# facebookresearch/habitat-lab

Measured on AMD Instinct MI355X. Metric: env-steps/sec (SPS) PointNav RGB-D 256x256, 64 envs x 128 rollout, higher is better.
Workload: dtype f32; 1 GPU; PointNav SimpleCNN+GRU, 64 envs x 128 steps, 256x256 RGB-D synthetic; envs_per_gpu=64, rollout_steps=128, ppo_epoch=4, num_mini_batch=4, parallelism=dp1

## Files before the change

habitat-lab_amd/csrc/conv2_dgrad_strip.h:

```cpp
#pragma once
#include "igemm_bf3.h"
#include "ops.h"

namespace hab {

struct C2dArgs {
    const float* dy;
    const float* wd;
    const float* mask;
    float* dx;
    int B;
    int strips, items;
    int sign_schedule;
    int H, W, Ho, Wo;
};

template <int R2>
struct C2dCfg {
    static constexpr int H = 63, Ho = 30, Wo = 30, NT = 512, CELLS = 32;
    static constexpr int YRS = R2 + 1, YCOLS = 33, YPIX = YRS * YCOLS;
    static constexpr int YU = YRS * Wo * 16, YPT = (YU + NT - 1) / NT;
    static constexpr int Y_PLANE = YPIX * 64;
    static constexpr int RED_LD = 68;
    static constexpr size_t Y_BYTES = ((size_t)3 * Y_PLANE * 2 + 15) / 16 * 16, RED_BYTES = (size_t)8 * 32 * RED_LD * 4;
// ... 98 lines not shown
#pragma unroll
                for (int v = 0; v < 16; ++v) acc[pw][v] = 0.f;
#pragma unroll
            for (int j = 0; j < 4; ++j) {
                const unsigned short* src = ys + pixidx * 64 + (((2 * j + hi) ^ swz) << 3);
                bf16x8 yf[3];
#pragma unroll
                for (int pl = 0; pl < 3; ++pl) yf[pl] = *reinterpret_cast<const bf16x8*>(src + pl * Cfg::Y_PLANE);
                constexpr int PA[6] = {2, 0, 1, 1, 0, 0}, PB[6] = {0, 2, 1, 0, 1, 0};
#pragma unroll
                for (int q = 0; q < 6; ++q)
#pragma unroll
                    for (int pw = 0; pw < 2; ++pw)
                        acc[pw] = __builtin_amdgcn_mfma_f32_32x32x16_bf16(bw[j][pw][PB[q]], yf[PA[q]], acc[pw], 0, 0, 0);
            }
            if (tr > 0) __syncthreads();
            float* mine = red + (size_t)(wave * 32 + li) * Cfg::RED_LD;
#pragma unroll
            for (int pw = 0; pw < 2; ++pw)
#pragma unroll
                for (int g = 0; g < 4; ++g)
                    *reinterpret_cast<f32x4*>(mine + pw * 32 + 8 * g + 4 * hi) =
                        f32x4{acc[pw][4 * g], acc[pw][4 * g + 1], acc[pw][4 * g + 2], acc[pw][4 * g + 3]};
            __syncthreads();
            const int h2 = h20 + tr;
#pragma unroll
            for (int q = 0; q < 2; ++q) {
                const int idx = t + q * NT, rph = idx >> 9, cell = (idx >> 4) & 31, cq = idx & 15;
                f32x4 s = *reinterpret_cast<const f32x4*>(red + (size_t)(rph * 32 + cell) * Cfg::RED_LD + cq * 4);
#pragma unroll
                for (int t4 = 1; t4 < 4; ++t4)
                    s += *reinterpret_cast<const f32x4*>(red + (size_t)((2 * t4 + rph) * 32 + cell) * Cfg::RED_LD + cq * 4);
                if (flip) s = -s;
                const int h = 2 * h2 + rph, w = 2 * cell + (cq >> 3);
                if (h < H && w < W) {
                    const size_t off = (((size_t)img * H + h) * W + w) * 32 + (cq & 7) * 4;
                    if (a.mask) {
                        const f32x4 m = mk[q];
#pragma unroll
                        for (int e = 0; e < 4; ++e) s[e] = m[e] > 0.f ? s[e] : 0.f;
                    }
                    *reinterpret_cast<f32x4*>(a.dx + off) = s;
                }
            }
        }
        __syncthreads();
    }
}

inline bool conv2_dgrad_strip_covers(const ConvDesc& d) {
    return d.KH == 4 && d.KW == 4 && d.stride == 2 && d.pad == 0 && d.C == 32 && d.Cout == 64 && d.H >= 4 && d.W >= 4 && d.H <= 63 && d.W <= 63;
}

inline int conv2_dgrad_strip(const ConvDesc& d, const float* dy, const float* wd, const float* mask, const float* add, float* dx,
                             hipStream_t stream) {
    if (!conv2_dgrad_strip_covers(d)) return HAB_NOT_APPLICABLE;
    if (add || d.B < 16 || !dy || !wd || !dx) return HAB_NOT_APPLICABLE;
    if ((reinterpret_cast<uintptr_t>(dy) | reinterpret_cast<uintptr_t>(wd) | reinterpret_cast<uintptr_t>(dx) | reinterpret_cast<uintptr_t>(mask)) & 15) return HAB_NOT_APPLICABLE;
    constexpr int R2 = 2;
    using Cfg = C2dCfg<R2>;
    C2dArgs a;
    a.dy = dy; a.wd = wd; a.mask = mask; a.dx = dx; a.B = d.B;
    a.H = d.H; a.W = d.W; a.Ho = (d.H - 4) / 2 + 1; a.Wo = (d.W - 4) / 2 + 1;
    a.strips = ((d.H + 1) / 2 + R2 - 1) / R2;
    if ((long long)d.B * a.strips > 0x7fffffffLL) return HAB_NOT_APPLICABLE;
    a.items = d.B * a.strips;
    a.sign_schedule = bf3_sign_schedule();
    static const hipError_t attr_err = [] {
        const hipError_t e0 = hipFuncSetAttribute(reinterpret_cast<const void*>(conv2_dgrad_strip_kernel<R2, false>),
                                                  hipFuncAttributeMaxDynamicSharedMemorySize, (int)Cfg::LDS_BYTES);
        const hipError_t e1 = hipFuncSetAttribute(reinterpret_cast<const void*>(conv2_dgrad_strip_kernel<R2, true>),
                                                  hipFuncAttributeMaxDynamicSharedMemorySize, (int)Cfg::LDS_BYTES);
        return e0 != hipSuccess ? e0 : e1;
    }();
    if (attr_err != hipSuccess) return (int)attr_err;
    int grid = 256;
    while (grid > 8 && grid > a.items) grid -= 8;
    if (d.H == 63 && d.W == 63) conv2_dgrad_strip_kernel<R2, false><<<grid, Cfg::NT, Cfg::LDS_BYTES, stream>>>(a);
    else conv2_dgrad_strip_kernel<R2, true><<<grid, Cfg::NT, Cfg::LDS_BYTES, stream>>>(a);
    HAB_LAUNCH_CHECK();
    return HAB_OK;
}

}
```

habitat-lab_amd/csrc/gemm_ops.hip:

```cpp
#include "igemm.h"
#include "igemm_dma.h"
#include "igemm_dma_wgrad.h"
#include "igemm_bf3.h"
#include "igemm_bf3_ws.h"
#include "dense_bf3.h"
#include "obs_conv_bf3.h"
#include "obs_conv_bf3_ws.h"
#include "obs_conv_patch.h"
#include "wgrad3x3_bf3.h"
#include "conv2_fwd_strip.h"
#include "conv2_dgrad_strip.h"
#include "obs_wgrad_bf3.h"
#include "obs_wgrad_strip.h"
#include "conv_patch_bf3.h"
#include "wgrad3x3_patch.h"
#include "prob_build.h"
#include <stdlib.h>

#include <atomic>

#include "../../include/habitat_amd.h"

namespace hab {

static std::atomic<int> g_bf3_mode{-1};
int matrix_path_bits() {
    int m = g_bf3_mode.load(std::memory_order_relaxed);
    if (m < 0) {
        static const int from_env = hab_env_int("HAB_BF3", MP_DEFAULT);
        int expected = -1;
        g_bf3_mode.compare_exchange_strong(expected, from_env, std::memory_order_relaxed);
        m = g_bf3_mode.load(std::memory_order_relaxed);
    }
    return m;
}
extern "C" int hab_set_matrix_path(int mode) {
    const int prev = matrix_path_bits();
    if (mode >= 0) g_bf3_mode.store(mode, std::memory_order_relaxed);
    return prev;
}

template <int TM_, int TN_, int WM_, int WN_>
struct Tile {
    static constexpr int TM = TM_, TN = TN_, WM = WM_, WN = WN_;
};
using Tile128x128 = Tile<2, 2, 2, 2>;
static bool rows_fit(int M, int rows, int other) { return M % rows == 0 || cdiv(M, rows) * rows < cdiv(M, other) * other; }
template <bool WG, class F>
static int by_width(int M, int N, F launch) {
    if (N <= 32) {
        if constexpr (WG) {
            if (rows_fit(M, 96, 256)) return launch(Tile<1, 1, 3, 1>{});
        }
        return launch(Tile<2, 1, 4, 1>{});
    }
    if (N <= 64) {
        if constexpr (WG) {
            if (rows_fit(M, 96, 128)) return launch(Tile<1, 2, 3, 1>{});
        }
        return launch(Tile<1, 2, 4, 1>{});
    }
    return launch(Tile128x128{});
}

// ... 31 lines not shown
        if (p.dma_ok() && p.M > 64 && p.N <= 128) return dma_launch<true>(p, ws, ws_floats, target_blocks, stream);
    }
    if (p.M <= 64) {
        if (p.N <= 32) return igemm_launch<P, 1, 1, 2, 1>(p, ws, ws_floats, target_blocks, stream);
        if (p.N <= 64) return igemm_launch<P, 1, 1, 2, 2>(p, ws, ws_floats, target_blocks, stream);
        return igemm_launch<P, 1, 2, 2, 2>(p, ws, ws_floats, target_blocks, stream);
    }
    return by_width<WG>(p.M, p.N, [&](auto t) {
        using T = decltype(t);
        return igemm_launch<P, T::TM, T::TN, T::WM, T::WN>(p, ws, ws_floats, target_blocks, stream);
    });
}

static bool patch3x3_wanted(const ConvDesc& d, int M) { return matrix_path_on(MP_PATCH3X3) && d.stride == 1 && d.KH == 3 && d.KW == 3 && M > 64; }
static PatchGeom patch3x3_geom(const float* in, int Hi, int Wi, int Ci, int Ho, int Wo, int off, int flip) {
    PatchGeom gq{};
    gq.in = in; gq.Hi = Hi; gq.Wi = Wi; gq.Ci = Ci; gq.Ho = Ho; gq.Wo = Wo; gq.KH = 3; gq.KW = 3;
    gq.off_h = off; gq.off_w = off; gq.flip = flip;
    return gq;
}

int conv_fwd(const ConvDesc& d, const float* x, const float* wf, const float* bias, float* y, int relu, float* ws,
             size_t ws_floats, hipStream_t stream) {
    ConvFwdProb p;
    HAB_TRY(build(p, d, x, wf, bias, y, relu));
    if (matrix_path_on(MP_CONV2_FWD | MP_RC))
        HAB_TRY_FORM(conv2_fwd_strip(p, ws, ws_floats, stream));
    if (patch3x3_wanted(d, p.M))
        HAB_TRY_FORM(conv_patch_bf3_dispatch(p, patch3x3_geom(x, d.H, d.W, d.C, p.g.Ho, p.g.Wo, -d.pad, 0), ws, ws_floats, stream));
    return run_igemm(p, ws, ws_floats, stream);
}
int64_t obs_conv_weight_image_floats() { return ((int64_t)OCP_W_ELEMS + 1) / 2 + 4; }
int obs_conv_weight_image(const float* wf, int Cout, int KH, int KW, int C, void* img, hipStream_t stream) {
    return obs_conv_patch_weight_image(wf, Cout, KH, KW, C, reinterpret_cast<unsigned short*>(img), stream);
}
int obs_conv_fwd(const ConvDesc& d, const ObsView& obs, const float* wf, const float* bias, float* y, int relu, float* ws,
                 size_t ws_floats, hipStream_t stream, const void* wimg) {
    ObsConvFwdProb p;
    HAB_TRY(build(p, d, obs, wf, bias, y, relu));
    if (matrix_path_on(MP_OBS_PATCH | MP_OBS) && p.quad)
        HAB_TRY_FORM(obs_conv_patch_launch(p, ws, ws_floats, stream, reinterpret_cast<const unsigned short*>(wimg)));
    if (matrix_path_on(MP_WS | MP_OBS) && p.quad && p.M > 64)
        HAB_TRY_FORM(obs_conv_bf3_ws_launch(p, ws, ws_floats, stream));
    if (matrix_path_on(MP_OBS) && p.quad && p.M > 64)
        HAB_TRY_FORM(obs_conv_bf3_launch<2>(p, ws, ws_floats, stream));
    return run_igemm(p, ws, ws_floats, stream);
}
__global__ void dgrad_empty_class_kernel(ConvDgradProb p) {
    const long long total = (long long)p.g.B * p.Hc * p.Wc * p.N;
    for (long long e = (long long)blockIdx.x * blockDim.x + threadIdx.x; e < total; e += (long long)gridDim.x * blockDim.x)
        p.store((int)(e / p.N), (int)(e % p.N), 0.f);
}

int conv_dgrad(const ConvDesc& d, const float* dy, const float* wd, const float* mask, const float* add, float* dx,
               float* ws, size_t ws_floats, hipStream_t stream) {
    if (matrix_path_on(MP_CONV2_DGRAD | MP_RC))
        HAB_TRY_FORM(conv2_dgrad_strip(d, dy, wd, mask, add, dx, stream));
    if (d.stride > 1) {
        ConvDgradMergedProb q;
        HAB_TRY(check_conv(d));
        q.g = make_geom(d);
        if (ConvDgradMergedProb::applicable(q.g)) {
            q.dy = dy; q.w = wd; q.mask = mask; q.add = add; q.dx = dx;
            q.finish();
            if (matrix_path_on(MP_RC) && q.M > 64)
                return by_width<false>(q.M, q.N, [&](auto t) { return bf3_launch<ConvDgradMergedProb, decltype(t)>(q, ws, ws_floats, 256, stream); });
            if (q.dma_ok()) return dma_launch<false>(q, ws, ws_floats, 1024, stream);
        }
    }
    for (int ph = 0; ph < d.stride; ++ph)
        for (int pw = 0; pw < d.stride; ++pw) {
            ConvDgradProb p;
            HAB_TRY(build(p, d, dy, wd, mask, add, dx, ph, pw));
            if (p.Hc <= 0 || p.Wc <= 0) continue;
            if (patch3x3_wanted(d, p.M) && p.K > 0) {
                const int rc = conv_patch_bf3_dispatch(p, patch3x3_geom(dy, p.g.Ho, p.g.Wo, d.Cout, d.H, d.W, d.pad - 2, 1), ws, ws_floats, stream);
                if (rc == HAB_OK) continue;
                if (rc != HAB_NOT_APPLICABLE) return rc;
            }
            if (p.K <= 0) {
                p.M = d.B * p.Hc * p.Wc;
                dgrad_empty_class_kernel<<<1024, 256, 0, stream>>>(p);
                HAB_LAUNCH_CHECK();
                continue;
            }
            HAB_TRY(run_igemm(p, ws, ws_floats, stream));
        }
    return HAB_OK;
}
int conv_wgrad(const ConvDesc& d, const float* x, const float* dy, float* dw_oihw, float* dbias, float* ws, size_t ws_floats,
               hipStream_t stream) {
    ConvWgradProb p;
    HAB_TRY(build(p, d, x, dy, dw_oihw, dbias));
    if (ws && matrix_path_on(MP_WGRAD_STRIP | MP_IJ_WGRAD) && wgrad3x3_bf3_shape(p))
        HAB_TRY_FORM(wgrad3x3_bf3(p, ws, ws_floats, stream));
    if (ws && !matrix_path_on(MP_IJ_WGRAD)) {
        ConvWgradProb q = p;
        q.colsum = nullptr;
        auto bias_grad = [&] { return dbias ? colsum(dy, p.N, p.K, p.N, dbias, 0, ws, ws_floats, stream) : HAB_OK; };
        if (wgrad3x3_patch_ok(p)) {
            HAB_TRY(bias_grad());
            return wgrad3x3_patch(q, ws, ws_floats, stream);
        }
        if (d.pad == 0 && p.N <= 32 && wgrad_dma_ok(q)) {
            HAB_TRY(bias_grad());
            if (rows_fit(q.M, 288, 256)) return igemm_dma_wgrad_launch<3, 3, 1>(q, ws, ws_floats, 1024, stream);
            return igemm_dma_wgrad_launch<2, 4, 1>(q, ws, ws_floats, 1024, stream);
        }
    }
    return run_igemm(p, ws, ws_floats, stream);
// ... 194 lines not shown
        const int c = (int)(e % ld);
        const long long r = e / ld;
        wp[e] = c < C ? w[r * C + c] : 0.f;
    }
}
int pad_rows(const float* w, float* wp, int R, int C, int ld, hipStream_t stream) {
    if (!w || !wp || R <= 0 || C <= 0 || ld < C) return HAB_ERR_ARG;
    const long long total = (long long)R * ld;
    pad_rows_kernel<<<(int)fmin(2048.0, (double)cdivl(total, 256)), 256, 0, stream>>>(w, wp, R, C, ld);
    HAB_LAUNCH_CHECK();
    return HAB_OK;
}
int transpose2d(const float* w, float* wt, int R, int C, hipStream_t stream) {
    if (!w || !wt || R <= 0 || C <= 0) return HAB_ERR_ARG;
    transpose_kernel<<<dim3(cdiv(C, 32), cdiv(R, 32)), dim3(32, 8), 0, stream>>>(w, wt, R, C);
    HAB_LAUNCH_CHECK();
    return HAB_OK;
}

}

using namespace hab;

static ConvDesc mk(int B, int H, int W, int C, int Cout, int KH, int KW, int stride, int pad) {
    ConvDesc d;
    d.B = B; d.H = H; d.W = W; d.C = C; d.Cout = Cout; d.KH = KH; d.KW = KW; d.stride = stride; d.pad = pad;
    return d;
}
static ObsView mkobs(const uint8_t* rgb, const float* depth, const int* rows, int H, int W) {
    ObsView o;
    o.rgb = rgb; o.depth = depth; o.rows = rows; o.H = H; o.W = W; o.C = (rgb ? 3 : 0) + (depth ? 1 : 0);
    return o;
}

extern "C" int hab_conv2d_fwd(const float* x, const float* w_fwd, const float* bias, float* y, int B, int H, int W, int C,
                              int Cout, int KH, int KW, int stride, int pad, int relu, float* ws, size_t ws_floats,
                              hipStream_t stream) {
    if (!x || !w_fwd || !y) return HAB_ERR_ARG;
    return conv_fwd(mk(B, H, W, C, Cout, KH, KW, stride, pad), x, w_fwd, bias, y, relu, ws, ws_floats, stream);
}
extern "C" int hab_obs_conv2d_fwd(const uint8_t* rgb, const float* depth, const int* rows, const float* w_fwd,
                                  const float* bias, float* y, int B, int H, int W, int Cout, int KH, int KW, int stride,
                                  int pad, int relu, float* ws, size_t ws_floats, hipStream_t stream) {
    if ((!rgb && !depth) || !w_fwd || !y) return HAB_ERR_ARG;
    ObsView o = mkobs(rgb, depth, rows, H, W);
    return obs_conv_fwd(mk(B, H, W, o.C, Cout, KH, KW, stride, pad), o, w_fwd, bias, y, relu, ws, ws_floats, stream);
}
extern "C" int hab_conv2d_dgrad(const float* dy, const float* w_dgrad, const float* relu_mask, const float* add, float* dx,
                                int B, int H, int W, int C, int Cout, int KH, int KW, int stride, int pad, float* ws,
                                size_t ws_floats, hipStream_t stream) {
    if (!dy || !w_dgrad || !dx) return HAB_ERR_ARG;
    return conv_dgrad(mk(B, H, W, C, Cout, KH, KW, stride, pad), dy, w_dgrad, relu_mask, add, dx, ws, ws_floats, stream);
}
extern "C" int hab_conv2d_wgrad(const float* x, const float* dy, float* dw_oihw, float* dbias, int B, int H, int W, int C, int Cout,
                                int KH, int KW, int stride, int pad, float* ws, size_t ws_floats, hipStream_t stream) {
    if (!x || !dy || !dw_oihw) return HAB_ERR_ARG;
    return conv_wgrad(mk(B, H, W, C, Cout, KH, KW, stride, pad), x, dy, dw_oihw, dbias, ws, ws_floats, stream);
}
extern "C" int hab_obs_conv2d_wgrad(const uint8_t* rgb, const float* depth, const int* rows, const float* dy, float* dw_oihw,
                                    float* dbias, int B, int H, int W, int Cout, int KH, int KW, int stride, int pad, float* ws,
                                    size_t ws_floats, hipStream_t stream) {
    if ((!rgb && !depth) || !dy || !dw_oihw) return HAB_ERR_ARG;
    ObsView o = mkobs(rgb, depth, rows, H, W);
    return obs_conv_wgrad(mk(B, H, W, o.C, Cout, KH, KW, stride, pad), o, dy, dw_oihw, dbias, ws, ws_floats, stream);
}
extern "C" int hab_obs_conv2d_wgrad_form(const uint8_t* rgb, const float* depth, const int* rows, const float* dy, float* dw_oihw,
                                         float* dbias, int B, int H, int W, int Cout, int KH, int KW, int stride, int pad, const float* ws,
                                         size_t ws_floats) {
    if ((!rgb && !depth) || !dy || !dw_oihw) return HAB_ERR_ARG;
    ObsView o = mkobs(rgb, depth, rows, H, W);
    ObsConvWgradProb p;
    const int r = build(p, mk(B, H, W, o.C, Cout, KH, KW, stride, pad), o, dy, dw_oihw, dbias);
    if (r != HAB_OK) return r;
    return choose_obs_wgrad(p, ws, ws_floats);
}
extern "C" int hab_linear_fwd(const float* x, int ldx, const float* w, int ldw, const float* bias, float* y, int ldy, int M,
                              int N, int K, int relu, int accumulate, float* ws, size_t ws_floats, hipStream_t stream) {
    return linear_fwd(x, ldx, w, ldw, bias, y, ldy, M, N, K, relu, accumulate, ws, ws_floats, stream);
}
extern "C" int hab_linear_dgrad(const float* dy, int lddy, const float* w, int ldw, const float* relu_mask, int ldmask,
                                float* dx, int lddx, int M, int n_in, int n_out, int accumulate, float* ws, size_t ws_floats,
                                hipStream_t stream) {
    return linear_dgrad(dy, lddy, w, ldw, relu_mask, ldmask, n_in, dx, lddx, M, n_in, n_out, accumulate, ws, ws_floats, stream);
}
extern "C" int hab_linear_wgrad(const float* dy, int lddy, const float* x, int ldx, float* dw, int lddw, int M, int n_out,
                                int n_in, int perm_c, int perm_hw, int accumulate, float* ws, size_t ws_floats,
                                hipStream_t stream) {
    return linear_wgrad(dy, lddy, x, ldx, dw, lddw, M, n_out, n_in, perm_c, perm_hw, accumulate, ws, ws_floats, stream);
}
extern "C" int hab_debug_dense_trace(long long* out320) {
    return (int)hipMemcpyFromSymbol(out320, HIP_SYMBOL(hab::dn_trace), sizeof(long long) * 8 * 8 * 5);
}
extern "C" int hab_colsum(const float* a, int lda, int M, int N, float* out, int accumulate, float* ws, size_t ws_floats,
                          hipStream_t stream) {
    return colsum(a, lda, M, N, out, accumulate, ws, ws_floats, stream);
}
extern "C" int hab_repack_conv_weight(const float* w_oihw, float* w_fwd, float* w_dgrad, int Cout, int Cin, int KH, int KW,
                                      int cin_padded, hipStream_t stream) {
    return repack_conv(w_oihw, w_fwd, w_dgrad, Cout, Cin, KH, KW, cin_padded, stream);
}
extern "C" int hab_repack_flatten_weight(const float* w, float* w_packed, int N, int C, int HW, hipStream_t stream) {
    return repack_flatten(w, w_packed, N, C, HW, stream);
}
extern "C" int hab_transpose2d(const float* w, float* wt, int R, int C, hipStream_t stream) {
    return transpose2d(w, wt, R, C, stream);
}
// ... 1 lines not shown
```

habitat-lab_amd/habitat_amd/_lib.py:

```python
from __future__ import annotations

import ctypes as C
import os
from ctypes import POINTER, c_char_p, c_double, c_float, c_int, c_int32, c_int64, c_size_t, c_uint8, c_uint32, c_void_p

_HERE = os.path.dirname(os.path.abspath(__file__))
LIB_PATH = os.path.join(_HERE, "libhabitat_amd.so")

vp = c_void_p
ALLREDUCE_FN = C.CFUNCTYPE(None, c_void_p, c_int, c_float, c_void_p)
GRAD_READY_FN = C.CFUNCTYPE(None, c_int64, c_int64, c_void_p)


class HabError(RuntimeError):
    pass


class PolicyDesc(C.Structure):
    _fields_ = [(n, c_int32) for n in (
        "arch", "backbone", "baseplanes", "normalize_visual_inputs", "rnn_type", "rnn_layers", "hidden", "num_actions",
        "H", "W", "has_rgb", "has_depth", "goal_dim", "max_frames", "max_envs", "visual_order", "has_semantic",
        "num_object_categories", "has_compass", "has_gps", "action_dist", "gauss_flags")] + [("gauss_min_std", c_float),
                                                                                                ("gauss_max_std", c_float),
                                                                                                ("pointgoal_dim", c_int32),
# ... 18 lines not shown
                ("gps", vp), ("visual_features", vp), ("pointgoal", vp), ("proximity", vp), ("visual", vp * 4), ("fused", vp * 8)]


class EmbedSlot(C.Structure):
    _fields_ = [("kind", c_int32), ("input", vp), ("weight", vp), ("bias", vp), ("d_weight", vp), ("d_bias", vp), ("num_tokens", c_int32)]


class PackInfo(C.Structure):
    _fields_ = [("select_inds", vp), ("frag_env", vp), ("frag_start", vp), ("step_offsets_host", vp),
                ("num_seqs_at_step_host", vp), ("P", c_int32), ("F", c_int32), ("max_len", c_int32), ("env_first_frame", vp)]


SIGNATURES = {
    "hab_abi_version": (c_int, []),
    "hab_error_string": (c_char_p, [c_int]),
    "hab_synth_step": (c_int, [vp, vp, vp, vp, vp, vp, vp, c_uint32, c_uint32, c_int, c_int, c_int, c_int, vp]),
    "hab_synth_objectnav_sensors": (c_int, [vp, vp, vp, vp, vp, c_uint32, c_uint32, c_int, c_int, c_int, vp]),
    "hab_nav2d_state_bytes": (c_int, []),
    "hab_nav2d_step": (c_int, [vp] * 13 + [c_uint32, c_uint32] + [c_int] * 7 + [vp]),
    "hab_nav2d_vel_step": (c_int, [vp] * 13 + [c_uint32, c_uint32] + [c_int] * 8 + [c_float, c_int, c_int, vp]),
    "hab_nav2d_geo_bytes": (c_int, []),
    "hab_nav2d_geo_build": (c_int, [vp, c_size_t, vp, vp, c_int, c_int, c_int, vp]),
    "hab_nav2d_step_geo": (c_int, [vp] * 14 + [c_uint32, c_uint32] + [c_int] * 7 + [vp]),
    "hab_nav2d_vel_step_geo": (c_int, [vp] * 14 + [c_uint32, c_uint32] + [c_int] * 8 + [c_float, c_int, c_int, vp]),
    "hab_nav2d_obj_state_bytes": (c_int, []),
    "hab_nav2d_obj_step": (c_int, [vp] * 17 + [c_uint32, c_uint32] + [c_int] * 10 + [vp]),
    "hab_nav2d_obj_geo_bytes": (c_int, []),
    "hab_nav2d_obj_geo_build": (c_int, [vp, c_size_t, vp, vp, c_int, c_int, c_int, c_int, vp]),
    "hab_nav2d_obj_step_geo": (c_int, [vp] * 18 + [c_uint32, c_uint32] + [c_int] * 10 + [vp]),
    "hab_nav2d_rearr_state_bytes": (c_int, []),
    "hab_nav2d_rearr_step": (c_int, [vp] * 15 + [c_uint32, c_uint32] + [c_int] * 8 + [vp]),
    "hab_obs_resize_crop": (c_int, [vp, vp, c_int, c_int, c_int, c_int, c_int, c_int, c_int, c_int, c_int, c_int, c_int, c_int, vp]),
    "hab_obs_resize_crop_form": (c_int, [vp, c_int, c_int, c_int, c_int, c_int, c_int, c_int, c_int]),
    "hab_obs_project": (c_int, [vp, c_int, vp, c_int, c_int, c_int, c_int, c_int, vp, vp, c_int, c_int, vp]),
    "hab_rollout_step_stats": (c_int, [vp, vp, vp, vp, vp, vp, vp, c_int, c_int, vp]),
    "hab_compute_returns": (c_int, [vp, vp, vp, vp, vp, c_int, c_int, c_float, c_float, c_int, c_int, vp]),
    "hab_advantages": (c_int, [vp, vp, vp, c_int, c_int, vp, vp, vp]),
    "hab_ppo_loss": (c_int, [vp, vp, vp, vp, vp, vp, vp, vp, c_int, c_float, c_float, c_float, c_int, vp, vp, vp, vp, vp]),
    "hab_ppo_loss_ver": (c_int, [vp, vp, vp, vp, vp, vp, vp, vp, c_int, c_float, c_float, c_float, c_int, vp, vp, vp, c_int64, vp, c_float,
                                 vp, vp, vp, vp, vp]),
    "hab_lagrange_adam_step": (c_int, [vp, vp, vp, vp, c_float, c_float, c_float, c_float, c_float, c_int, c_float, c_float, vp, vp]),
    "hab_ver_compute_returns": (c_int, [vp, vp, vp, vp, vp, vp, vp, vp, c_int, c_double, c_double, vp]),
    "hab_ver_is_coeffs": (c_int, [vp, c_int, c_int, c_int, vp, vp, vp]),
    "hab_clip_adam_step": (c_int, [vp, vp, vp, vp, c_size_t, vp, c_int, c_float, c_float, c_float, c_float, c_float,
                                   c_float, c_int, vp, vp]),
    "hab_sample_actions": (c_int, [vp, vp, vp, c_int, c_int, c_int, vp]),
    "hab_set_matrix_path": (c_int, [c_int]),
    "hab_conv2d_fwd": (c_int, [vp, vp, vp, vp] + [c_int] * 10 + [vp, c_size_t, vp]),
    "hab_obs_conv2d_fwd": (c_int, [vp, vp, vp, vp, vp, vp] + [c_int] * 9 + [vp, c_size_t, vp]),
    "hab_conv2d_dgrad": (c_int, [vp, vp, vp, vp, vp] + [c_int] * 9 + [vp, c_size_t, vp]),
    "hab_conv2d_wgrad": (c_int, [vp, vp, vp, vp] + [c_int] * 9 + [vp, c_size_t, vp]),
    "hab_obs_conv2d_wgrad": (c_int, [vp, vp, vp, vp, vp, vp] + [c_int] * 8 + [vp, c_size_t, vp]),
    "hab_obs_conv2d_wgrad_form": (c_int, [vp, vp, vp, vp, vp, vp] + [c_int] * 8 + [vp, c_size_t]),
    "hab_linear_fwd": (c_int, [vp, c_int, vp, c_int, vp, vp, c_int, c_int, c_int, c_int, c_int, c_int, vp, c_size_t, vp]),
    "hab_linear_dgrad": (c_int, [vp, c_int, vp, c_int, vp, c_int, vp, c_int, c_int, c_int, c_int, c_int, vp, c_size_t, vp]),
    "hab_linear_wgrad": (c_int, [vp, c_int, vp, c_int, vp, c_int, c_int, c_int, c_int, c_int, c_int, c_int, vp, c_size_t, vp]),
    "hab_colsum": (c_int, [vp, c_int, c_int, c_int, vp, c_int, vp, c_size_t, vp]),
    "hab_repack_conv_weight": (c_int, [vp, vp, vp, c_int, c_int, c_int, c_int, c_int, vp]),
    "hab_repack_flatten_weight": (c_int, [vp, vp, c_int, c_int, c_int, vp]),
    "hab_transpose2d": (c_int, [vp, vp, c_int, c_int, vp]),
    "hab_obs_ingest_pool": (c_int, [vp, vp, vp, vp, vp, c_int, c_int, c_int, c_int, c_int, c_int, c_int, vp]),
    "hab_obs_ingest_pool_sensors": (c_int, [vp, vp, vp, vp, c_int, vp, vp, c_int, c_int, c_int, c_int, vp, vp, vp, vp, vp, vp]),
    "hab_fused_gather": (c_int, [vp, vp, c_int, vp, vp, c_int, c_int, c_int, c_int, c_int, vp]),
    "hab_channel_moments": (c_int, [vp, c_int64, c_int, c_int, vp, vp, vp, c_int, vp]),
    "hab_running_mean_var_update": (c_int, [vp, vp, vp, vp, vp, c_float, c_int, vp]),
    "hab_running_mean_var_normalize": (c_int, [vp, c_int64, c_int, c_int, vp, vp, vp]),
    "hab_groupnorm_fwd": (c_int, [vp, vp, vp, vp, vp, vp, vp, c_int, c_int, c_int, c_int, c_int, c_float, vp, c_int64, vp]),
    "hab_groupnorm_bwd": (c_int, [vp, vp, vp, vp, vp, vp, vp, vp, vp, c_int, c_int, c_int, c_int, vp, c_int64, vp]),
    "hab_split_weight_planes": (c_int, [vp, c_int, c_int, vp, vp]),
    "hab_stem_split_weights": (c_int, [vp, vp, vp]),
    "hab_stem_conv_wgrad": (c_int, [vp, vp, vp, c_int, c_int, c_int, c_int, vp, c_size_t, vp, vp]),
    "hab_stem_conv_fwd": (c_int, [vp, vp, vp, c_int, c_int, c_int, vp, vp, c_int, vp]),
    "hab_conv_gn_fwd": (c_int, [vp] * 9 + [c_int] * 11 + [c_float, vp]),
    "hab_maxpool3x3s2_fwd": (c_int, [vp, vp, vp, c_int, c_int, c_int, c_int, vp]),
    "hab_maxpool3x3s2_bwd": (c_int, [vp, vp, vp, c_int, c_int, c_int, c_int, vp]),
    "hab_nav_embed_fwd": (c_int, [POINTER(EmbedSlot), c_int, vp, vp, vp, c_int, c_int, c_int, vp, vp]),
    "hab_nav_embed_bwd": (c_int, [POINTER(EmbedSlot), c_int, vp, vp, c_int, c_int, c_int, vp, c_size_t, vp]),
    "hab_build_pack_info": (c_int, [vp, c_int, c_int] + [vp] * 12),
    "hab_build_pack_info_from_ids": (c_int, [vp, vp, vp, c_int] + [vp] * 11),
    "hab_policy_create": (c_int, [POINTER(PolicyDesc), POINTER(vp)]),
    "hab_policy_destroy": (None, [vp]),
    "hab_policy_num_params": (c_int, [vp]),
    "hab_policy_param_info": (c_int, [vp, c_int, c_char_p, c_int, POINTER(c_int64), POINTER(c_int), POINTER(c_int64)]),
    "hab_policy_param_is_buffer": (c_int, [vp, c_int]),
    "hab_policy_set_training": (c_int, [vp, c_int]),
    "hab_comm_available": (c_int, []),
    "hab_comm_unique_id": (c_int, [vp]),
    "hab_comm_create": (c_int, [vp, c_int, c_int, vp]),
    "hab_comm_destroy": (None, [vp]),
    "hab_comm_world_size": (c_int, [vp]),
    "hab_comm_allreduce_sum": (c_int, [vp, vp, c_int64, vp]),
    "hab_policy_set_comm": (c_int, [vp, vp]),
    "hab_policy_grad_sync": (c_int, [vp, vp]),
    "hab_policy_set_grad_ready": (c_int, [vp, GRAD_READY_FN, vp]),
    "hab_policy_set_allreduce": (c_int, [vp, ALLREDUCE_FN, vp, c_int]),
    "hab_policy_param_floats": (c_int64, [vp]),
    "hab_policy_packed_floats": (c_int64, [vp]),
    "hab_policy_work_floats": (c_int64, [vp]),
    "hab_policy_bind": (c_int, [vp, vp, vp, vp, vp, c_int64]),
    "hab_policy_repack": (c_int, [vp, vp]),
    "hab_policy_encode": (c_int, [vp, POINTER(Obs), c_int, vp, vp]),
    "hab_policy_visual_feature_shape": (c_int, [vp, POINTER(c_int), POINTER(c_int), POINTER(c_int)]),
    "hab_policy_act": (c_int, [vp, POINTER(Obs), vp, vp, vp, c_int, c_int, vp, vp, vp, vp, vp, vp]),
    "hab_policy_evaluate": (c_int, [vp, POINTER(Obs), vp, vp, c_int, vp, vp, POINTER(PackInfo), c_int, c_int, vp, vp, vp, vp]),
    "hab_policy_final_hidden": (c_int, [vp, vp, vp]),
    "hab_policy_set_extra_grads": (c_int, [vp, vp, vp]),
# ... 46 lines not shown
```

include/habitat_amd.h:

```cpp
#ifndef HABITAT_AMD_H
#define HABITAT_AMD_H

#include <stddef.h>
#include <stdint.h>

#ifdef __cplusplus
extern "C" {
#endif

#ifndef __HIP_PLATFORM_AMD__
typedef struct ihipStream_t* hipStream_t;
#endif

#define HAB_ABI_VERSION 1
int hab_abi_version(void);
const char* hab_error_string(int code);

int hab_synth_step(uint8_t* rgb , float* depth , float* goal , float* reward ,
                   uint8_t* not_done , int64_t* env_t , int64_t* since_reset , uint32_t seed,
                   uint32_t env_offset, int N, int H, int W, int advance, hipStream_t stream);
int hab_synth_objectnav_sensors(int32_t* semantic, int64_t* objectgoal, float* compass, float* gps, const int64_t* env_t,
                                uint32_t seed, uint32_t env_offset, int N, int H, int W, hipStream_t stream);

#define HAB_NAV2D_STATE_BYTES 224
// ... 124 lines not shown
#define HAB_ADV_EXT_NORMALIZE 3
#define HAB_ADV_STATS_VAR 4
int hab_advantages(const float* returns, const float* value_preds, float* adv, int count, int mode,
                   const float* ext_stats, float* stats_out, hipStream_t stream);

int hab_ppo_loss(const float* values, const float* logp, const float* entropy, const float* old_logp,
                 const float* adv, const float* old_values, const float* returns, const int* rows, int B,
                 float clip_param, float value_loss_coef, float entropy_coef, int use_clipped_value_loss,
                 float* d_value, float* d_logp, float* d_entropy, float* out12, hipStream_t stream);

int hab_ppo_loss_ver(const float* values, const float* logp, const float* entropy, const float* old_logp, const float* adv,
                     const float* old_values, const float* returns, const int* rows, int B, float clip_param, float value_loss_coef,
                     float entropy_coef, int use_clipped_value_loss, const float* is_coeffs, const uint8_t* is_stale,
                     const int64_t* policy_version, int64_t current_policy_version, const float* log_alpha, float entropy_threshold,
                     float* d_value, float* d_logp, float* d_entropy, float* out20, hipStream_t stream);
int hab_lagrange_adam_step(float* log_alpha, float* exp_avg, float* exp_avg_sq, const float* grad, float grad_scale, float lr, float beta1,
                           float beta2, float eps, int step, float log_alpha_min, float log_alpha_max,
                           float* alpha_out , hipStream_t stream);

int hab_ver_compute_returns(const float* rewards, const float* value_preds, const uint8_t* is_stale, float* returns,
                            const int32_t* select_inds, const int32_t* step_offsets, const int32_t* sequence_lengths,
                            const uint8_t* last_sequence_in_batch_mask, int F, double gamma, double tau, hipStream_t stream);
int hab_ver_is_coeffs(const int64_t* environment_ids, int n, int num_envs, int num_steps, int32_t* counts_scratch, float* is_coeffs,
                      hipStream_t stream);

int hab_clip_adam_step(float* params, const float* grads, float* exp_avg, float* exp_avg_sq, size_t n,
                       double* scratch_partials, int scratch_len, float grad_scale, float max_grad_norm, float lr,
                       float beta1, float beta2, float eps, int step, float* grad_norm_out, hipStream_t stream);

int hab_sample_actions(const float* probs, const float* exp_noise, int64_t* actions, int n, int A, int deterministic,
                       hipStream_t stream);

int hab_set_matrix_path(int mode);

int hab_conv2d_fwd(const float* x, const float* w_fwd, const float* bias, float* y, int B, int H, int W, int C, int Cout,
                   int KH, int KW, int stride, int pad, int relu, float* ws, size_t ws_floats, hipStream_t stream);
int hab_obs_conv2d_fwd(const uint8_t* rgb, const float* depth, const int* rows, const float* w_fwd, const float* bias,
                       float* y, int B, int H, int W, int Cout, int KH, int KW, int stride, int pad, int relu, float* ws,
                       size_t ws_floats, hipStream_t stream);
int hab_conv2d_dgrad(const float* dy, const float* w_dgrad, const float* relu_mask, const float* add, float* dx, int B,
                     int H, int W, int C, int Cout, int KH, int KW, int stride, int pad, float* ws, size_t ws_floats,
                     hipStream_t stream);
int hab_conv2d_wgrad(const float* x, const float* dy, float* dw_oihw, float* dbias, int B, int H, int W, int C, int Cout,
                     int KH, int KW, int stride, int pad, float* ws, size_t ws_floats, hipStream_t stream);
int hab_obs_conv2d_wgrad(const uint8_t* rgb, const float* depth, const int* rows, const float* dy, float* dw_oihw,
                         float* dbias, int B, int H, int W, int Cout, int KH, int KW, int stride, int pad, float* ws,
                         size_t ws_floats, hipStream_t stream);
#define HAB_OBS_WGRAD_FORM_IGEMM 0
#define HAB_OBS_WGRAD_FORM_IM2COL 1
#define HAB_OBS_WGRAD_FORM_STRIP 2
int hab_obs_conv2d_wgrad_form(const uint8_t* rgb, const float* depth, const int* rows, const float* dy, float* dw_oihw,
                              float* dbias, int B, int H, int W, int Cout, int KH, int KW, int stride, int pad, const float* ws,
                              size_t ws_floats);
int hab_linear_fwd(const float* x, int ldx, const float* w, int ldw, const float* bias, float* y, int ldy, int M, int N,
                   int K, int relu, int accumulate, float* ws, size_t ws_floats, hipStream_t stream);
int hab_linear_dgrad(const float* dy, int lddy, const float* w, int ldw, const float* relu_mask, int ldmask, float* dx,
                     int lddx, int M, int n_in, int n_out, int accumulate, float* ws, size_t ws_floats,
                     hipStream_t stream);
int hab_linear_wgrad(const float* dy, int lddy, const float* x, int ldx, float* dw, int lddw, int M, int n_out, int n_in,
                     int perm_c, int perm_hw, int accumulate, float* ws, size_t ws_floats, hipStream_t stream);
int hab_colsum(const float* a, int lda, int M, int N, float* out, int accumulate, float* ws, size_t ws_floats,
               hipStream_t stream);
int hab_repack_conv_weight(const float* w_oihw, float* w_fwd, float* w_dgrad, int Cout, int Cin, int KH, int KW,
                           int cin_padded, hipStream_t stream);
int hab_repack_flatten_weight(const float* w, float* w_packed, int N, int C, int HW, hipStream_t stream);
int hab_transpose2d(const float* w, float* wt, int R, int C, hipStream_t stream);

int hab_obs_ingest_pool(const uint8_t* rgb, const float* depth, const int32_t* semantic, const int* rows, float* y, int B, int H, int W,
                        int cpad, int c_rgb, int c_depth, int c_sem ,
                        hipStream_t stream);
int hab_obs_ingest_pool_sensors(const void* const* sensors, const int32_t* dtypes, const int32_t* channels, const float* scales, int n,
                                const int* rows, float* y, int B, int H, int W, int cpad, const float* norm_mean, const float* norm_var,
                                const float* pivot, double* mom_partial, int* mom_blocks, hipStream_t stream);
int hab_fused_gather(const float* const* sensors, const int32_t* widths, int n, const int* rows, float* dst, int ld, int col0, int pad0,
                     int npad, int B, hipStream_t stream);
int hab_channel_moments(const float* x, int64_t npix, int cpad, int mode, const float* mean, float* out, double* scratch,
                        int scratch_len, hipStream_t stream);
int hab_running_mean_var_update(float* r_mean, float* r_var, float* r_count, const float* b_mean, const float* b_var, float n, int C,
                                hipStream_t stream);
int hab_running_mean_var_normalize(float* x, int64_t npix, int cpad, int C, const float* mean, const float* var, hipStream_t stream);
int hab_groupnorm_fwd(const float* x, float* y, const float* gamma, const float* beta, const float* residual, float* mean,
                      float* rstd, int B, int HW, int C, int groups, int relu, float eps, float* ws, int64_t ws_floats,
                      hipStream_t stream);
int hab_groupnorm_bwd(const float* x, const float* dy, const float* relu_out, float* dx, float* dy_masked, const float* gamma,
                      const float* mean, const float* rstd, float* chan_sums, int B, int HW, int C, int groups, float* ws,
                      int64_t ws_floats, hipStream_t stream);
int hab_split_weight_planes(const float* w_fwd, int Cout, int K, uint16_t* planes, hipStream_t stream);
int hab_stem_split_weights(const float* w_fwd, uint16_t* planes, hipStream_t stream);
int hab_stem_conv_fwd(const float* x, const uint16_t* w_planes, float* y, int B, int H, int W, const float* norm, float* gn_part, int gn_groups,
                      hipStream_t stream);
int hab_stem_conv_wgrad(const float* x, const float* dy, float* dw_oihw, int B, int H, int W, int creal, float* ws, size_t ws_floats,
                        const float* norm, hipStream_t stream);
int hab_conv_gn_fwd(const float* x, const uint16_t* w_planes, const float* gamma, const float* beta, const float* residual, float* y,
                    float* raw, float* mean, float* rstd, int B, int H, int W, int C, int Cout, int KH, int KW, int stride, int pad,
                    int groups, int relu, float eps, hipStream_t stream);
int hab_maxpool3x3s2_fwd(const float* x, float* y, uint8_t* idx, int B, int H, int W, int C, hipStream_t stream);
int hab_maxpool3x3s2_bwd(const float* dy, const uint8_t* idx, float* dx, int B, int H, int W, int C, hipStream_t stream);
#define HAB_EMB_POLAR 0
#define HAB_EMB_TOKEN 1
#define HAB_EMB_COSSIN 2
#define HAB_EMB_LIN2 3
#define HAB_EMB_PREV 4
#define HAB_EMB_PREVLIN 5
#define HAB_EMB_LINN 6
typedef struct hab_embed_slot {
    int32_t kind;
// ... 182 lines not shown
```

Before: 63940 env-steps/s.

## Add strip-tiled MFMA dgrad kernel for the 3x3 stride-1 conv3 layer

Adds a dedicated dgrad kernel for the 3x3/stride-1, 64-to-32-channel conv layer. It stages dy row strips in LDS as three-way bf16-split planes, plus a sign-flipped copy for the sign schedule, and accumulates the nine taps with 32x32x16 bf16 MFMA across two wave groups that hand off partial sums through LDS. Work is distributed through per-XCD atomic draw counters taken from a device-side slot pool, replacing the generic implicit-GEMM dgrad path for this layer. It also factors out the applicability checks and exposes a form query, at the cost of extra code complexity and device-counter reset logic.

```diff
diff --git a/habitat-lab_amd/csrc/conv2_dgrad_strip.h b/habitat-lab_amd/csrc/conv2_dgrad_strip.h
--- a/habitat-lab_amd/csrc/conv2_dgrad_strip.h
+++ b/habitat-lab_amd/csrc/conv2_dgrad_strip.h
@@ -174,18 +174,23 @@
     return d.KH == 4 && d.KW == 4 && d.stride == 2 && d.pad == 0 && d.C == 32 && d.Cout == 64 && d.H >= 4 && d.W >= 4 && d.H <= 63 && d.W <= 63;
 }
 
+constexpr int C2D_CELL_ROWS = 2;
+inline bool conv2_dgrad_strip_serves(const ConvDesc& d, const float* dy, const float* wd, const float* mask, const float* add, const float* dx) {
+    if (!conv2_dgrad_strip_covers(d)) return false;
+    if (add || d.B < 16 || !dy || !wd || !dx) return false;
+    if ((reinterpret_cast<uintptr_t>(dy) | reinterpret_cast<uintptr_t>(wd) | reinterpret_cast<uintptr_t>(dx) | reinterpret_cast<uintptr_t>(mask)) & 15) return false;
+    return (long long)d.B * cdiv((d.H + 1) / 2, C2D_CELL_ROWS) <= 0x7fffffffLL;
+}
+
 inline int conv2_dgrad_strip(const ConvDesc& d, const float* dy, const float* wd, const float* mask, const float* add, float* dx,
                              hipStream_t stream) {
-    if (!conv2_dgrad_strip_covers(d)) return HAB_NOT_APPLICABLE;
-    if (add || d.B < 16 || !dy || !wd || !dx) return HAB_NOT_APPLICABLE;
-    if ((reinterpret_cast<uintptr_t>(dy) | reinterpret_cast<uintptr_t>(wd) | reinterpret_cast<uintptr_t>(dx) | reinterpret_cast<uintptr_t>(mask)) & 15) return HAB_NOT_APPLICABLE;
-    constexpr int R2 = 2;
+    if (!conv2_dgrad_strip_serves(d, dy, wd, mask, add, dx)) return HAB_NOT_APPLICABLE;
+    constexpr int R2 = C2D_CELL_ROWS;
     using Cfg = C2dCfg<R2>;
     C2dArgs a;
     a.dy = dy; a.wd = wd; a.mask = mask; a.dx = dx; a.B = d.B;
     a.H = d.H; a.W = d.W; a.Ho = (d.H - 4) / 2 + 1; a.Wo = (d.W - 4) / 2 + 1;
-    a.strips = ((d.H + 1) / 2 + R2 - 1) / R2;
-    if ((long long)d.B * a.strips > 0x7fffffffLL) return HAB_NOT_APPLICABLE;
+    a.strips = cdiv((d.H + 1) / 2, R2);
     a.items = d.B * a.strips;
     a.sign_schedule = bf3_sign_schedule();
     static const hipError_t attr_err = [] {
diff --git a/habitat-lab_amd/csrc/conv3_dgrad_strip.h b/habitat-lab_amd/csrc/conv3_dgrad_strip.h
--- /dev/null
+++ b/habitat-lab_amd/csrc/conv3_dgrad_strip.h
@@ -0,0 +1,241 @@
+#pragma once
+#include "igemm_bf3.h"
+#include "ops.h"
+
+#include <atomic>
+
+namespace hab {
+
+struct C3dArgs {
+    const float* dy;
+    const float* wd;
+    const float* mask;
+    float* dx;
+    int B;
+    int strips, items;
+    int sign_schedule;
+    int H, W, Ho, Wo;
+    unsigned* ctr;
+};
+
+constexpr int C3D_DRAW_SLOTS = 64;
+__device__ unsigned c3d_draw_pool[C3D_DRAW_SLOTS * 16];
+
+template <int R>
+struct C3dCfg {
+    static constexpr int H = 30, Ho = 28, Wo = 28, NT = 512, MAXWO = 30;
+    static constexpr int YRS = R + 2, YCOLS = 34, YPIX = YRS * YCOLS;
+    static constexpr int YU = YRS * Wo * 8, YPT = (YRS * MAXWO * 8 + NT - 1) / NT;
+    static constexpr int Y_PLANE = YPIX * 32;
+    static constexpr int Y_COPY = 3 * Y_PLANE;
+    static constexpr size_t Y_BYTES = (size_t)2 * Y_COPY * 2, PASS_BYTES = (size_t)2 * 4 * 16 * 64 * 4;
+    static constexpr size_t LDS_BYTES = Y_BYTES + PASS_BYTES;
+    static_assert(R % 2 == 0, "the waves take the rows of a strip in pairs");
+    static_assert((Y_COPY * 2) % 256 == 0, "both copies on the same banks");
+};
+
+template <int R, bool RT>
+__global__ void __launch_bounds__(512) conv3_dgrad_strip_kernel(const C3dArgs a) {
+    using Cfg = C3dCfg<R>;
+    constexpr int NT = Cfg::NT;
+    const int H = RT ? a.H : Cfg::H, W = RT ? a.W : Cfg::H, Ho = RT ? a.Ho : Cfg::Ho, Wo = RT ? a.Wo : Cfg::Wo;
+    const int YU = Cfg::YRS * Wo * 8;
+    extern __shared__ __attribute__((aligned(16))) unsigned short smem16[];
+    unsigned short* ys = smem16;
+    f32x4* pass = reinterpret_cast<f32x4*>(reinterpret_cast<char*>(smem16) + Cfg::Y_BYTES);
+    const int t = threadIdx.x, lane = t & 63;
+    const int wave = __builtin_amdgcn_readfirstlane(t >> 6);
+    const int rsel = wave & 1, chalf = (wave >> 1) & 1, z = wave >> 2;
+    const int li = lane & 31, hi = lane >> 5;
+
+    __shared__ int s_draw[2];
+    const int xcd = blockIdx.x & 7;
+    const int per_xcd = (a.items + 7) >> 3, run0 = xcd * per_xcd, run_len = max(0, min(a.items, run0 + per_xcd) - run0);
+    if (t == 0) { s_draw[0] = (int)atomicAdd(a.ctr + xcd, 1u); s_draw[1] = (int)atomicAdd(a.ctr + xcd, 1u); }
+
+    for (int i = t; i < (int)(Cfg::Y_BYTES / 16); i += NT) reinterpret_cast<u32x4*>(smem16)[i] = u32x4{0u, 0u, 0u, 0u};
+
+    bf16x8 bw[9][3];
+    int tapoff[9];
+#pragma unroll
+    for (int j = 0; j < 9; ++j) {
+        const int s = 9 * z + j, tap = s >> 1, coh = s & 1, kh = tap / 3, kw = tap - 3 * kh;
+        tapoff[j] = (2 - kh) * Cfg::YCOLS + 2 - kw;
+        const float* src = a.wd + ((size_t)(chalf * 32 + li) * 9 + tap) * 32 + coh * 16 + hi * 8;
+        const f32x4 v0 = *reinterpret_cast<const f32x4*>(src), v1 = *reinterpret_cast<const f32x4*>(src + 4);
+        unsigned p[3][4];
+        bf3_split2(v0[0], v0[1], p[0][0], p[1][0], p[2][0]);
+        bf3_split2(v0[2], v0[3], p[0][1], p[1][1], p[2][1]);
+        bf3_split2(v1[0], v1[1], p[0][2], p[1][2], p[2][2]);
+        bf3_split2(v1[2], v1[3], p[0][3], p[1][3], p[2][3]);
+#pragma unroll
+        for (int pl = 0; pl < 3; ++pl) bw[j][pl] = __builtin_bit_cast(bf16x8, u32x4{p[pl][0], p[pl][1], p[pl][2], p[pl][3]});
+    }
+
+    f32x4 yr[Cfg::YPT];
+    int pf_h0 = 0;
+    auto fetch = [&](int item) {
+        const int img = item / a.strips, h0 = (item - img * a.strips) * R;
+        pf_h0 = h0;
+#pragma unroll
+        for (int j = 0; j < Cfg::YPT; ++j) {
+            const int u = t + j * NT;
+            const int r = u / (Wo * 8), row = h0 - 2 + r;
+            const bool ok = u < YU && (unsigned)row < (unsigned)Ho;
+            const size_t off = ok ? ((size_t)img * Ho + row) * (size_t)(Wo * 32) + (size_t)(u - r * (Wo * 8)) * 4 : 0;
+            yr[j] = *reinterpret_cast<const f32x4*>(a.dy + off);
+        }
+    };
+    auto stage = [&]() {
+#pragma unroll
+        for (int j = 0; j < Cfg::YPT; ++j) {
+            const int u = t + j * NT;
+            if (u >= YU) continue;
+            const int r = u / (Wo * 8), rem = u - r * (Wo * 8), w = rem >> 3, c4 = rem & 7;
+            const int pixidx = r * Cfg::YCOLS + w + 2;
+            unsigned short* dst = ys + pixidx * 32 + (((c4 >> 1) ^ ((pixidx >> 2) & 3)) << 3) + (c4 & 1) * 4;
+            const bool in_image = (unsigned)(pf_h0 - 2 + r) < (unsigned)Ho;
+            const f32x4 v = in_image ? yr[j] : f32x4{0.f, 0.f, 0.f, 0.f};
+            unsigned w0[3], w1[3];
+            bf3_split2(v[0], v[1], w0[0], w0[1], w0[2]);
+            bf3_split2(v[2], v[3], w1[0], w1[1], w1[2]);
+#pragma unroll
+            for (int pl = 0; pl < 3; ++pl) {
+                *reinterpret_cast<u32x2*>(dst + pl * Cfg::Y_PLANE) = u32x2{w0[pl], w1[pl]};
+                *reinterpret_cast<u32x2*>(dst + Cfg::Y_COPY + pl * Cfg::Y_PLANE) = u32x2{w0[pl] ^ 0x80008000u, w1[pl] ^ 0x80008000u};
+            }
+        }
+    };
+
+    __syncthreads();
+    int cur = s_draw[0], nxt = s_draw[1];
+    if (cur < run_len) fetch(run0 + cur);
+    for (int it = 0; cur < run_len; ++it) {
+        const int item = run0 + cur;
+        stage();
+        __syncthreads();
+        const bool more = nxt < run_len;
+        if (more) fetch(run0 + nxt);
+        if (more && t == 0) s_draw[it & 1] = (int)atomicAdd(a.ctr + xcd, 1u);
+        const int img = item / a.strips, h0 = (item - img * a.strips) * R;
+#pragma unroll 1
+        for (int ph = 0; ph <= R / 2; ++ph) {
+            const int rp = ph - z;
+            if (rp >= 0 && rp < R / 2) {
+                const int tr = 2 * rp + rsel, h = h0 + tr;
+                const bool live = h < H && li < W;
+                const size_t out = (((size_t)img * H + h) * W + li) * 64 + chalf * 32 + 4 * hi;
+                const bool flip = a.sign_schedule && ((((img * H + h) * W + li) >> 7) & 1);
+                f32x4 mk[4];
+                if (z == 1 && a.mask) {
+#pragma unroll
+                    for (int g = 0; g < 4; ++g) mk[g] = *reinterpret_cast<const f32x4*>(a.mask + (live ? out + 8 * g : (size_t)0));
+                }
+                const int pix0 = tr * Cfg::YCOLS + li;
+                const unsigned short* ysl = ys + (flip ? Cfg::Y_COPY : 0);
+                f32x4* hand = pass + (size_t)((((ph - z) & 1) * 4 + (wave & 3)) * 4) * 64 + lane;
+                f32x16 acc;
+                if (z == 0) {
+#pragma unroll
+                    for (int v = 0; v < 16; ++v) acc[v] = 0.f;
+                } else {
+#pragma unroll
+                    for (int g = 0; g < 4; ++g) {
+                        const f32x4 q = hand[g * 64];
+                        acc[4 * g] = q[0]; acc[4 * g + 1] = q[1]; acc[4 * g + 2] = q[2]; acc[4 * g + 3] = q[3];
+                    }
+                }
+                bf16x8 yf[2][3];
+                auto read_frags = [&](int j, bf16x8* f) {
+                    const int pixidx = pix0 + tapoff[j];
+                    const int chunk = 2 * ((9 * z + j) & 1) + hi;
+                    const unsigned short* src = ysl + pixidx * 32 + ((chunk ^ ((pixidx >> 2) & 3)) << 3);
+#pragma unroll
+                    for (int pl = 0; pl < 3; ++pl) f[pl] = *reinterpret_cast<const bf16x8*>(src + pl * Cfg::Y_PLANE);
+                };
+                read_frags(0, yf[0]);
+#pragma unroll
+                for (int j = 0; j < 9; ++j) {
+                    if (j + 1 < 9) read_frags(j + 1, yf[(j + 1) & 1]);
+                    __builtin_amdgcn_sched_barrier(0);
+                    constexpr int PA[6] = {2, 0, 1, 1, 0, 0}, PB[6] = {0, 2, 1, 0, 1, 0};
+#pragma unroll
+                    for (int q = 0; q < 6; ++q)
+                        acc = __builtin_amdgcn_mfma_f32_32x32x16_bf16(bw[j][PB[q]], yf[j & 1][PA[q]], acc, 0, 0, 0);
+                    __builtin_amdgcn_sched_barrier(0);
+                }
+                if (z == 0) {
+#pragma unroll
+                    for (int g = 0; g < 4; ++g) hand[g * 64] = f32x4{acc[4 * g], acc[4 * g + 1], acc[4 * g + 2], acc[4 * g + 3]};
+                } else if (live) {
+#pragma unroll
+                    for (int g = 0; g < 4; ++g) {
+                        f32x4 s = f32x4{acc[4 * g], acc[4 * g + 1], acc[4 * g + 2], acc[4 * g + 3]};
+                        if (flip) s = -s;
+                        if (a.mask) {
+#pragma unroll
+                            for (int e = 0; e < 4; ++e) s[e] = mk[g][e] > 0.f ? s[e] : 0.f;
+                        }
+                        *reinterpret_cast<f32x4*>(a.dx + out + 8 * g) = s;
+                    }
+                }
+            }
+            __syncthreads();
+        }
+        cur = nxt;
+        nxt = more ? s_draw[it & 1] : run_len;
+    }
+    if (t == 0) {
+        __threadfence();
+        if (atomicAdd(a.ctr + 8, 1u) == gridDim.x - 1) {
+#pragma unroll
+            for (int i = 0; i < 9; ++i) a.ctr[i] = 0u;
+        }
+    }
+}
+
+inline bool conv3_dgrad_strip_covers(const ConvDesc& d) {
+    return d.KH == 3 && d.KW == 3 && d.stride == 1 && d.pad == 0 && d.C == 64 && d.Cout == 32 && d.H >= 3 && d.W >= 3 && d.W <= 32;
+}
+constexpr int C3D_ROWS = 6;
+inline bool conv3_dgrad_strip_serves(const ConvDesc& d, const float* dy, const float* wd, const float* mask, const float* add, const float* dx) {
+    if (!conv3_dgrad_strip_covers(d)) return false;
+    if (add || d.B < 16 || !dy || !wd || !dx) return false;
+    if ((reinterpret_cast<uintptr_t>(dy) | reinterpret_cast<uintptr_t>(wd) | reinterpret_cast<uintptr_t>(dx) | reinterpret_cast<uintptr_t>(mask)) & 15) return false;
+    if ((long long)d.B * d.H * d.W > 0x7fffffffLL) return false;
+    return (long long)d.B * cdiv(d.H, C3D_ROWS) <= 0x7fffffffLL;
+}
+
+inline int conv3_dgrad_strip(const ConvDesc& d, const float* dy, const float* wd, const float* mask, const float* add, float* dx,
+                             hipStream_t stream) {
+    if (!conv3_dgrad_strip_serves(d, dy, wd, mask, add, dx)) return HAB_NOT_APPLICABLE;
+    constexpr int R = C3D_ROWS;
+    using Cfg = C3dCfg<R>;
+    C3dArgs a;
+    a.dy = dy; a.wd = wd; a.mask = mask; a.dx = dx; a.B = d.B;
+    a.H = d.H; a.W = d.W; a.Ho = d.H - 2; a.Wo = d.W - 2;
+    a.strips = cdiv(d.H, R);
+    a.items = d.B * a.strips;
+    a.sign_schedule = bf3_sign_schedule();
+    static std::atomic<unsigned> next_slot{0};
+    static unsigned* pool = nullptr;
+    static const hipError_t sym_err = hipGetSymbolAddress(reinterpret_cast<void**>(&pool), HIP_SYMBOL(c3d_draw_pool));
+    if (sym_err != hipSuccess || !pool) return HAB_ERR_ARG;
+    a.ctr = pool + (size_t)(next_slot.fetch_add(1, std::memory_order_relaxed) % C3D_DRAW_SLOTS) * 16;
+    static const hipError_t attr_err = [] {
+        const hipError_t e0 = hipFuncSetAttribute(reinterpret_cast<const void*>(conv3_dgrad_strip_kernel<R, false>),
+                                                  hipFuncAttributeMaxDynamicSharedMemorySize, (int)Cfg::LDS_BYTES);
+        const hipError_t e1 = hipFuncSetAttribute(reinterpret_cast<const void*>(conv3_dgrad_strip_kernel<R, true>),
+                                                  hipFuncAttributeMaxDynamicSharedMemorySize, (int)Cfg::LDS_BYTES);
+        return e0 != hipSuccess ? e0 : e1;
+    }();
+    if (attr_err != hipSuccess) return (int)attr_err;
+    int grid = 256;
+    while (grid > 8 && grid > a.items) grid -= 8;
+    if (d.H == Cfg::H && d.W == Cfg::H) conv3_dgrad_strip_kernel<R, false><<<grid, Cfg::NT, Cfg::LDS_BYTES, stream>>>(a);
+    else conv3_dgrad_strip_kernel<R, true><<<grid, Cfg::NT, Cfg::LDS_BYTES, stream>>>(a);
+    HAB_LAUNCH_CHECK();
+    return HAB_OK;
+}
+
+}
diff --git a/habitat-lab_amd/csrc/gemm_ops.hip b/habitat-lab_amd/csrc/gemm_ops.hip
--- a/habitat-lab_amd/csrc/gemm_ops.hip
+++ b/habitat-lab_amd/csrc/gemm_ops.hip
@@ -10,6 +10,7 @@
 #include "wgrad3x3_bf3.h"
 #include "conv2_fwd_strip.h"
 #include "conv2_dgrad_strip.h"
+#include "conv3_dgrad_strip.h"
 #include "obs_wgrad_bf3.h"
 #include "obs_wgrad_strip.h"
 #include "conv_patch_bf3.h"
@@ -147,10 +148,17 @@
         p.store((int)(e / p.N), (int)(e % p.N), 0.f);
 }
 
+static int choose_conv_dgrad(const ConvDesc& d, const float* dy, const float* wd, const float* mask, const float* add, const float* dx) {
+    if (!matrix_path_on(MP_CONV2_DGRAD | MP_RC)) return HAB_CONV_DGRAD_FORM_GENERAL;
+    if (conv2_dgrad_strip_serves(d, dy, wd, mask, add, dx)) return HAB_CONV_DGRAD_FORM_CONV2_STRIP;
+    if (conv3_dgrad_strip_serves(d, dy, wd, mask, add, dx)) return HAB_CONV_DGRAD_FORM_CONV3_STRIP;
+    return HAB_CONV_DGRAD_FORM_GENERAL;
+}
 int conv_dgrad(const ConvDesc& d, const float* dy, const float* wd, const float* mask, const float* add, float* dx,
                float* ws, size_t ws_floats, hipStream_t stream) {
-    if (matrix_path_on(MP_CONV2_DGRAD | MP_RC))
-        HAB_TRY_FORM(conv2_dgrad_strip(d, dy, wd, mask, add, dx, stream));
+    const int form = choose_conv_dgrad(d, dy, wd, mask, add, dx);
+    if (form == HAB_CONV_DGRAD_FORM_CONV2_STRIP) HAB_TRY_FORM(conv2_dgrad_strip(d, dy, wd, mask, add, dx, stream));
+    if (form == HAB_CONV_DGRAD_FORM_CONV3_STRIP) HAB_TRY_FORM(conv3_dgrad_strip(d, dy, wd, mask, add, dx, stream));
     if (d.stride > 1) {
         ConvDgradMergedProb q;
         HAB_TRY(check_conv(d));
@@ -451,6 +459,16 @@
     if (!dy || !w_dgrad || !dx) return HAB_ERR_ARG;
     return conv_dgrad(mk(B, H, W, C, Cout, KH, KW, stride, pad), dy, w_dgrad, relu_mask, add, dx, ws, ws_floats, stream);
 }
+extern "C" int hab_conv2d_dgrad_form(const float* dy, const float* w_dgrad, const float* relu_mask, const float* add, float* dx,
+                                     int B, int H, int W, int C, int Cout, int KH, int KW, int stride, int pad, const float* ws,
+                                     size_t ws_floats) {
+    (void)ws; (void)ws_floats;
+    if (!dy || !w_dgrad || !dx) return HAB_ERR_ARG;
+    const ConvDesc d = mk(B, H, W, C, Cout, KH, KW, stride, pad);
+    const int r = check_conv(d);
+    if (r != HAB_OK) return r;
+    return choose_conv_dgrad(d, dy, w_dgrad, relu_mask, add, dx);
+}
 extern "C" int hab_conv2d_wgrad(const float* x, const float* dy, float* dw_oihw, float* dbias, int B, int H, int W, int C, int Cout,
                                 int KH, int KW, int stride, int pad, float* ws, size_t ws_floats, hipStream_t stream) {
     if (!x || !dy || !dw_oihw) return HAB_ERR_ARG;
diff --git a/habitat-lab_amd/habitat_amd/_lib.py b/habitat-lab_amd/habitat_amd/_lib.py
--- a/habitat-lab_amd/habitat_amd/_lib.py
+++ b/habitat-lab_amd/habitat_amd/_lib.py
@@ -94,6 +94,7 @@
     "hab_conv2d_wgrad": (c_int, [vp, vp, vp, vp] + [c_int] * 9 + [vp, c_size_t, vp]),
     "hab_obs_conv2d_wgrad": (c_int, [vp, vp, vp, vp, vp, vp] + [c_int] * 8 + [vp, c_size_t, vp]),
     "hab_obs_conv2d_wgrad_form": (c_int, [vp, vp, vp, vp, vp, vp] + [c_int] * 8 + [vp, c_size_t]),
+    "hab_conv2d_dgrad_form": (c_int, [vp, vp, vp, vp, vp] + [c_int] * 9 + [vp, c_size_t]),
     "hab_linear_fwd": (c_int, [vp, c_int, vp, c_int, vp, vp, c_int, c_int, c_int, c_int, c_int, c_int, vp, c_size_t, vp]),
     "hab_linear_dgrad": (c_int, [vp, c_int, vp, c_int, vp, c_int, vp, c_int, c_int, c_int, c_int, c_int, vp, c_size_t, vp]),
     "hab_linear_wgrad": (c_int, [vp, c_int, vp, c_int, vp, c_int, c_int, c_int, c_int, c_int, c_int, c_int, vp, c_size_t, vp]),
diff --git a/include/habitat_amd.h b/include/habitat_amd.h
--- a/include/habitat_amd.h
+++ b/include/habitat_amd.h
@@ -200,6 +200,11 @@
 int hab_obs_conv2d_wgrad_form(const uint8_t* rgb, const float* depth, const int* rows, const float* dy, float* dw_oihw,
                               float* dbias, int B, int H, int W, int Cout, int KH, int KW, int stride, int pad, const float* ws,
                               size_t ws_floats);
+#define HAB_CONV_DGRAD_FORM_GENERAL 0
+#define HAB_CONV_DGRAD_FORM_CONV2_STRIP 1
+#define HAB_CONV_DGRAD_FORM_CONV3_STRIP 2
+int hab_conv2d_dgrad_form(const float* dy, const float* w_dgrad, const float* relu_mask, const float* add, float* dx, int B,
+                          int H, int W, int C, int Cout, int KH, int KW, int stride, int pad, const float* ws, size_t ws_floats);
 int hab_linear_fwd(const float* x, int ldx, const float* w, int ldw, const float* bias, float* y, int ldy, int M, int N,
                    int K, int relu, int accumulate, float* ws, size_t ws_floats, hipStream_t stream);
 int hab_linear_dgrad(const float* dy, int lddy, const float* w, int ldw, const float* relu_mask, int ldmask, float* dx,
```

Measured after the change: 65050 env-steps/s (median of 6 runs). 1.02x the previous value.
